# gabrielspmoreira/chameleon_recsys

Hardware: AMD Instinct MI355X
Metric: NAR training sessions/sec (higher is better)
Workload: dtype f32

## Files before the change

### chameleon_recsys_amd/csrc/dm_fused.hip

```cpp
#include "gemm_shared.h"
#include <type_traits>

#define DMF_NT 2
#define DMF_COLS (32 * DMF_NT)
#define DMF_PLANE (DMF_COLS * 128)
#define DMF_HALF (3 * DMF_PLANE)
#define DMF_RED_OFF (2 * DMF_HALF)
#define DMF_RED_BYTES (8 * 4 * DMF_COLS * 4)

static_assert(DMF_NT == 2, "the epilogue packs exactly two tiles' columns per lane");

struct DmfParams {
    const float* dS1; int lds1;
    const __bf16* W; long long w_ps;
    const float* Z2c; const float* pred;
    __bf16* out; long long out_ps;
    const H2Scale* osc;
    const H2Scale* sa; const H2Scale* sw;
    float* dpred; float* b2part;
    int C, BT, NC, PW;
    int out_blocked;
};

__device__ __forceinline__ void dmf_dma_one(unsigned lds, unsigned voff, const u32x4& r) {
    unsigned keep;
    asm volatile(
        "s_nop 4\n\t"
        "s_mov_b32 %0, m0\n\t"
        "s_mov_b32 m0, %1\n\ts_nop 0\n\tbuffer_load_dwordx4 %2, %3, 0 offen lds\n\t"
        "s_mov_b32 m0, %0"
        : "=&s"(keep) : "s"(lds), "v"(voff), "s"(r) : "memory");
}

template <int MODE>
__global__ __launch_bounds__(512) void k_dm_mulpred_fused(DmfParams p) {
    constexpr bool H2 = MODE == 1 || MODE == 3, B16 = MODE == 2, F16P = MODE == 3;
    constexpr int NPL = B16 ? 1 : (F16P ? 2 : 3);
    extern __shared__ __attribute__((aligned(1024))) unsigned char dmf_smem[];
    const int lane = threadIdx.x & 63, wave = __builtin_amdgcn_readfirstlane(threadIdx.x >> 6);
    const int l31 = lane & 31, hh = lane >> 5;
    const int NC = p.NC, C = p.C;
    const int pos0 = blockIdx.x * p.PW;
    const int npos = min(p.PW, p.BT - pos0);
    const int rows_valid = npos * NC;
    const size_t row0 = (size_t)pos0 * NC;
    const int wr0 = 32 * wave;

    bf16x8 AH[8], AM[(B16 || F16P) ? 1 : 8], AL[B16 ? 1 : 8];
    float ginv_a = 1.f, ginv_w = 1.f;
    if constexpr (B16) {
        const __bf16* a16 = reinterpret_cast<const __bf16*>(p.dS1);
        const __amdgpu_buffer_rsrc_t aw = __builtin_amdgcn_make_buffer_rsrc(const_cast<__bf16*>(a16 + row0 * (size_t)p.lds1), 0,
                                                                            (unsigned)((size_t)rows_valid * p.lds1 * 2), 0x00020000);
        const unsigned ao = ((unsigned)(wr0 + l31) * (unsigned)p.lds1 + 8u * hh) * 2u;
#pragma unroll
        for (int s = 0; s < 8; ++s) AH[s] = __builtin_bit_cast(bf16x8, __builtin_amdgcn_raw_buffer_load_b128(aw, ao + 32u * s, 0, 0));
    } else {
        const __amdgpu_buffer_rsrc_t aw = __builtin_amdgcn_make_buffer_rsrc(const_cast<float*>(p.dS1 + row0 * (size_t)p.lds1), 0,
                                                                            (unsigned)((size_t)rows_valid * p.lds1 * 4), 0x00020000);
        const unsigned ao = ((unsigned)(wr0 + l31) * (unsigned)p.lds1 + 8u * hh) * 4u;
        u32x4 x[16];
#pragma unroll
        for (int s = 0; s < 8; ++s) {
            x[2 * s] = __builtin_amdgcn_raw_buffer_load_b128(aw, ao + 64u * s, 0, 0);
            x[2 * s + 1] = __builtin_amdgcn_raw_buffer_load_b128(aw, ao + 64u * s + 16u, 0, 0);
        }
#pragma unroll
        for (int s = 0; s < 8; ++s) {
            const float v[8] = {__uint_as_float(x[2 * s].x), __uint_as_float(x[2 * s].y), __uint_as_float(x[2 * s].z), __uint_as_float(x[2 * s].w),
                                __uint_as_float(x[2 * s + 1].x), __uint_as_float(x[2 * s + 1].y), __uint_as_float(x[2 * s + 1].z),
                                __uint_as_float(x[2 * s + 1].w)};
            if constexpr (F16P) {
                const float sa = p.sa->scale;
#pragma unroll
                for (int e = 0; e < 8; ++e) {
                    _Float16 a, c;
                    split2h(v[e] * sa, a, c);
                    AH[s][e] = __builtin_bit_cast(__bf16, a); AL[s][e] = __builtin_bit_cast(__bf16, c);
                }
            } else {
#pragma unroll
                for (int e = 0; e < 8; ++e) { __bf16 a, b, c; split3(v[e], a, b, c); AH[s][e] = a; AM[s][e] = b; AL[s][e] = c; }
            }
        }
    }
    const __amdgpu_buffer_rsrc_t zw = B16 ?
        __builtin_amdgcn_make_buffer_rsrc(const_cast<__bf16*>(reinterpret_cast<const __bf16*>(p.Z2c) + row0 * (size_t)C), 0,
                                          (unsigned)((size_t)rows_valid * C * 2), 0x00020000) :
        __builtin_amdgcn_make_buffer_rsrc(const_cast<float*>(p.Z2c + row0 * (size_t)C), 0, (unsigned)((size_t)rows_valid * C * 4), 0x00020000);
    __amdgpu_buffer_rsrc_t ow[3];
#pragma unroll
    for (int q = 0; q < 3; ++q)
        ow[q] = __builtin_amdgcn_make_buffer_rsrc(p.out + ((H2 && q == 2) || B16 ? 0 : q) * p.out_ps + row0 * (size_t)C, 0, (unsigned)((size_t)rows_valid * C * 2), 0x00020000);
    const bool oblk = H2 && p.out_blocked != 0;
    const unsigned rin = (unsigned)(row0 & 255), tile_bytes = ((unsigned)C >> 5) * (unsigned)(H2B_BLOCK * 2);
    if (oblk) {
#pragma unroll
        for (int q = 0; q < 2; ++q)
            ow[q] = __builtin_amdgcn_make_buffer_rsrc(p.out + q * p.out_ps + (row0 >> 8) * (size_t)((unsigned)C >> 5) * H2B_BLOCK, 0, 2u * tile_bytes, 0x00020000);
    }
    float osc = 1.f;
    if constexpr (H2) osc = p.osc->scale;
    if constexpr (F16P) { ginv_a = p.sa->inv; ginv_w = p.sw->inv; }

    typedef __attribute__((address_space(3))) unsigned char lds_u8;
    const unsigned lds_base = (unsigned)(unsigned long long)(lds_u8*)dmf_smem;
    u32x4 rw[3];
#pragma unroll
    for (int q = 0; q < 3; ++q) {
        const unsigned long long a = (unsigned long long)(p.W + q * p.w_ps);
        rw[q].x = (unsigned)a; rw[q].y = (unsigned)(a >> 32) & 0xFFFFu; rw[q].z = (unsigned)((size_t)C * 128 * 2); rw[q].w = 0x00020000u;
    }
    unsigned voff;
    {
        const int slot = 8 * wave + (lane >> 3);
        const int piece = (lane & 7) ^ ((slot >> 1) & 7);
        const int col = DMF_NT * (slot & 31) + (slot >> 5);
        voff = (unsigned)(col * 128 + piece * 8) * 2u;
    }
    auto dma_half = [&](int h) {
        const unsigned base = lds_base + (unsigned)(h & 1) * DMF_HALF + (unsigned)wave * 1024u;
        const unsigned add = (unsigned)(((h >> 1) * DMF_COLS) * 128 + (h & 1) * 64) * 2u;
#pragma unroll
        for (int q = 0; q < NPL; ++q) dmf_dma_one(base + (unsigned)q * DMF_PLANE, voff + add, rw[q]);
    };
    unsigned fo[4];
#pragma unroll
    for (int t = 0; t < 4; ++t) fo[t] = (unsigned)(l31 * 128 + (((2 * t + hh) ^ ((l31 >> 1) & 7)) * 16));

    const int pa = wr0 / NC;
    const int bnd = (pa + 1) * NC - wr0;
    const int ntiles = C / DMF_COLS, nhalf = 2 * ntiles;

    dma_half(0);
    dma_half(1);
    floatx16 acc[DMF_NT];
#pragma unroll
    for (int j = 0; j < DMF_NT; ++j)
#pragma unroll
        for (int e = 0; e < 16; ++e) acc[j][e] = 0.f;
    if constexpr (B16) asm volatile("s_waitcnt vmcnt(1)" ::: "memory");
    else if constexpr (F16P) asm volatile("s_waitcnt vmcnt(2)" ::: "memory");
    else asm volatile("s_waitcnt vmcnt(3)" ::: "memory");
    __builtin_amdgcn_fence(__ATOMIC_RELEASE, "workgroup", "local");
    __builtin_amdgcn_s_barrier();
    __builtin_amdgcn_fence(__ATOMIC_ACQUIRE, "workgroup", "local");

    auto mfma_half = [&](auto PARC) {
        constexpr int PAR = decltype(PARC)::value, s0 = PAR * 4;
        const unsigned char* S = dmf_smem + PAR * DMF_HALF;
        __builtin_amdgcn_sched_barrier(0);
#pragma unroll
        for (int t = 0; t < 4; ++t) {
            bf16x8 bh[DMF_NT], bm[DMF_NT], bl[DMF_NT];
#pragma unroll
            for (int j = 0; j < DMF_NT; ++j) {
                bh[j] = *reinterpret_cast<const bf16x8*>(S + fo[t] + j * 4096);
                if constexpr (F16P) {
                    bl[j] = *reinterpret_cast<const bf16x8*>(S + DMF_PLANE + fo[t] + j * 4096);
                } else if constexpr (!B16) {
                    bm[j] = *reinterpret_cast<const bf16x8*>(S + DMF_PLANE + fo[t] + j * 4096);
                    bl[j] = *reinterpret_cast<const bf16x8*>(S + 2 * DMF_PLANE + fo[t] + j * 4096);
                }
            }
            if constexpr (F16P) {
                typedef _Float16 dmf_half8 __attribute__((ext_vector_type(8)));
#pragma unroll
                for (int j = 0; j < DMF_NT; ++j)
                    acc[j] = __builtin_amdgcn_mfma_f32_32x32x16_f16(__builtin_bit_cast(dmf_half8, AL[s0 + t]), __builtin_bit_cast(dmf_half8, bh[j]), acc[j], 0, 0, 0);
#pragma unroll
                for (int j = 0; j < DMF_NT; ++j)
                    acc[j] = __builtin_amdgcn_mfma_f32_32x32x16_f16(__builtin_bit_cast(dmf_half8, AH[s0 + t]), __builtin_bit_cast(dmf_half8, bl[j]), acc[j], 0, 0, 0);
#pragma unroll
                for (int j = 0; j < DMF_NT; ++j)
                    acc[j] = __builtin_amdgcn_mfma_f32_32x32x16_f16(__builtin_bit_cast(dmf_half8, AH[s0 + t]), __builtin_bit_cast(dmf_half8, bh[j]), acc[j], 0, 0, 0);
            } else if constexpr (B16) {
#pragma unroll
                for (int j = 0; j < DMF_NT; ++j) acc[j] = __builtin_amdgcn_mfma_f32_32x32x16_bf16(AH[s0 + t], bh[j], acc[j], 0, 0, 0);
            } else {
#pragma unroll
                for (int j = 0; j < DMF_NT; ++j) acc[j] = __builtin_amdgcn_mfma_f32_32x32x16_bf16(AL[s0 + t], bh[j], acc[j], 0, 0, 0);
#pragma unroll
                for (int j = 0; j < DMF_NT; ++j) acc[j] = __builtin_amdgcn_mfma_f32_32x32x16_bf16(AH[s0 + t], bl[j], acc[j], 0, 0, 0);
#pragma unroll
                for (int j = 0; j < DMF_NT; ++j) acc[j] = __builtin_amdgcn_mfma_f32_32x32x16_bf16(AM[s0 + t], bm[j], acc[j], 0, 0, 0);
#pragma unroll
                for (int j = 0; j < DMF_NT; ++j) acc[j] = __builtin_amdgcn_mfma_f32_32x32x16_bf16(AM[s0 + t], bh[j], acc[j], 0, 0, 0);
#pragma unroll
                for (int j = 0; j < DMF_NT; ++j) acc[j] = __builtin_amdgcn_mfma_f32_32x32x16_bf16(AH[s0 + t], bm[j], acc[j], 0, 0, 0);
#pragma unroll
                for (int j = 0; j < DMF_NT; ++j) acc[j] = __builtin_amdgcn_mfma_f32_32x32x16_bf16(AH[s0 + t], bh[j], acc[j], 0, 0, 0);
            }
        }
    };
    for (int h = 0; h < nhalf; ++h) {
        if (h & 1) mfma_half(std::integral_constant<int, 1>{});
        else mfma_half(std::integral_constant<int, 0>{});
        __builtin_amdgcn_sched_barrier(0);
        asm volatile("s_waitcnt vmcnt(0)" ::: "memory");
        if (h & 1) {
            const int col = (h >> 1) * DMF_COLS + DMF_NT * l31;
            float2 pra = make_float2(0.f, 0.f), prb = pra;
            if (pa < npos) pra = *reinterpret_cast<const float2*>(p.pred + (size_t)(pos0 + pa) * C + col);
            if (pa + 1 < npos) prb = *reinterpret_cast<const float2*>(p.pred + (size_t)(pos0 + pa + 1) * C + col);
            float2 sa = make_float2(0.f, 0.f), sb = sa, ca = sa, cb = sa;
            typedef unsigned int u32x2_t __attribute__((ext_vector_type(2)));
            u32x2_t zz[16];
#pragma unroll
            for (int e = 0; e < 16; ++e) {
                const unsigned r = (unsigned)(wr0 + (e & 3) + 8 * (e >> 2) + 4 * hh);
                if constexpr (B16) {
                    const unsigned u = __builtin_amdgcn_raw_buffer_load_b32(zw, (r * (unsigned)C + (unsigned)col) * 2u, 0, 0);
                    zz[e].x = u << 16; zz[e].y = u & 0xFFFF0000u;
                } else {
                    zz[e] = __builtin_amdgcn_raw_buffer_load_b64(zw, (r * (unsigned)C + (unsigned)col) * 4u, 0, 0);
                }
            }
#pragma unroll
            for (int e = 0; e < 16; ++e) {
                const int rr = (e & 3) + 8 * (e >> 2) + 4 * hh;
                const unsigned r = (unsigned)(wr0 + rr);
                const float2 z = make_float2(__uint_as_float(zz[e].x), __uint_as_float(zz[e].y));
                const bool second = rr >= bnd;
                const float2 pr = second ? prb : pra;
                float2 g = make_float2(acc[0][e], acc[1][e]);
                if constexpr (F16P) { g.x = (g.x * ginv_a) * ginv_w; g.y = (g.y * ginv_a) * ginv_w; }
                if constexpr (B16) { g.x = (float)(__bf16)g.x; g.y = (float)(__bf16)g.y; }
                float2 o;
                o.x = g.x * pr.x * (1.f - z.x * z.x); o.y = g.y * pr.y * (1.f - z.y * z.y);
                if constexpr (B16) {
                    typedef __bf16 bf16x2_t __attribute__((ext_vector_type(2)));
                    bf16x2_t ph; ph[0] = (__bf16)o.x; ph[1] = (__bf16)o.y;
                    __builtin_amdgcn_raw_buffer_store_b32(__builtin_bit_cast(unsigned, ph), ow[0], (r * (unsigned)C + (unsigned)col) * 2u, 0, 0);
                    o.x = (float)ph[0]; o.y = (float)ph[1];
                } else if constexpr (H2) {
                    _Float16 h0, l0, h1, l1;
                    split2h(o.x * osc, h0, l0); split2h(o.y * osc, h1, l1);
                    const unsigned ph = (unsigned)h2_keep_sign(h0, o.x) | ((unsigned)h2_keep_sign(h1, o.y) << 16);
                    const unsigned pl = (unsigned)__builtin_bit_cast(unsigned short, l0) | ((unsigned)__builtin_bit_cast(unsigned short, l1) << 16);
                    unsigned oo = (r * (unsigned)C + (unsigned)col) * 2u;
                    if (oblk) {
                        const unsigned lr = rin + r;
                        oo = (int)r < rows_valid ? (lr >> 8) * tile_bytes + ((unsigned)col >> 5) * (unsigned)(H2B_BLOCK * 2) + (lr & 255u) * 64u + ((unsigned)col & 31u) * 2u
                                                 : 0x80000000u;
                    }
                    __builtin_amdgcn_raw_buffer_store_b32(ph, ow[0], oo, 0, 0);
                    __builtin_amdgcn_raw_buffer_store_b32(pl, ow[1], oo, 0, 0);
                } else {
                    typedef __bf16 bf16x2_t __attribute__((ext_vector_type(2)));
                    bf16x2_t ph, pm, pl;
                    __bf16 a, b, c;
                    split3(o.x, a, b, c); ph[0] = a; pm[0] = b; pl[0] = c;
                    split3(o.y, a, b, c); ph[1] = a; pm[1] = b; pl[1] = c;
                    const unsigned oo = (r * (unsigned)C + (unsigned)col) * 2u;
                    __builtin_amdgcn_raw_buffer_store_b32(__builtin_bit_cast(unsigned, ph), ow[0], oo, 0, 0);
                    __builtin_amdgcn_raw_buffer_store_b32(__builtin_bit_cast(unsigned, pm), ow[1], oo, 0, 0);
                    __builtin_amdgcn_raw_buffer_store_b32(__builtin_bit_cast(unsigned, pl), ow[2], oo, 0, 0);
                }
                const float2 gz = make_float2(g.x * z.x, g.y * z.y);
                sb.x += second ? gz.x : 0.f; sb.y += second ? gz.y : 0.f; cb.x += second ? o.x : 0.f; cb.y += second ? o.y : 0.f;
                sa.x += second ? 0.f : gz.x; sa.y += second ? 0.f : gz.y; ca.x += second ? 0.f : o.x; ca.y += second ? 0.f : o.y;
                acc[0][e] = 0.f; acc[1][e] = 0.f;
            }
            float* red = reinterpret_cast<float*>(dmf_smem + DMF_RED_OFF) + (size_t)wave * (4 * DMF_COLS);
            float2 q[4] = {sa, ca, sb, cb};
#pragma unroll
            for (int i = 0; i < 4; ++i) {
                float2 o;
                o.x = __shfl_xor(q[i].x, 32, 64); o.y = __shfl_xor(q[i].y, 32, 64);
                if (hh == 0) *reinterpret_cast<float2*>(red + i * DMF_COLS + DMF_NT * l31) = make_float2(q[i].x + o.x, q[i].y + o.y);
            }
        }
        __builtin_amdgcn_fence(__ATOMIC_RELEASE, "workgroup", "local");
        __builtin_amdgcn_s_waitcnt(0xc07f);
        __builtin_amdgcn_s_barrier();
        __builtin_amdgcn_fence(__ATOMIC_ACQUIRE, "workgroup", "local");
        if (h & 1) {
            const float* redw = reinterpret_cast<const float*>(dmf_smem + DMF_RED_OFF);
            for (int idx = threadIdx.x; idx < npos * DMF_COLS; idx += 512) {
                const int pl = idx / DMF_COLS, c = idx % DMF_COLS;
                float s = 0.f, cs = 0.f;
                const int w_lo = (pl * NC) >> 5, w_hi = min(7, ((pl + 1) * NC - 1) >> 5);
                for (int w = w_lo; w <= w_hi; ++w) {
                    const int slot = (pl == (32 * w) / NC) ? 0 : 1;
                    s += redw[(size_t)w * (4 * DMF_COLS) + slot * (2 * DMF_COLS) + c];
                    cs += redw[(size_t)w * (4 * DMF_COLS) + slot * (2 * DMF_COLS) + DMF_COLS + c];
                }
                const int colg = (h >> 1) * DMF_COLS + c;
                const float pr = p.pred[(size_t)(pos0 + pl) * C + colg];
                p.dpred[(size_t)(pos0 + pl) * C + colg] = s * (1.f - pr * pr);
                if (p.b2part) p.b2part[(size_t)(pos0 + pl) * C + colg] = cs;
            }
        }
        if (h + 2 < nhalf) dma_half(h + 2);
    }
    asm volatile("s_waitcnt vmcnt(0)" ::: "memory");
}

template <int MODE>
static int dm_mulpred_launch(const float* dS1, int lds1, int K, const void* Wp, long long w_plane_stride, const float* Z2c,
                             const float* pred, int C, int BT, int N, void* dZ2p, long long out_plane_stride, const void* out_scale_rec,
                             float* dpred_pre, float* col_part, void* stream, const void* a_scale_rec = nullptr, const void* w_scale_rec = nullptr,
                             int out_blocked = 0) {
    if (!dS1 || !Wp || !Z2c || !pred || !dZ2p || !dpred_pre || BT < 0 || N < 0 || ((MODE == 1 || MODE == 3) && !out_scale_rec)) return -CHAM_ERR_ARG;
    if (MODE == 3 && (!a_scale_rec || !w_scale_rec || (((uintptr_t)a_scale_rec | (uintptr_t)w_scale_rec) & 3))) return -CHAM_ERR_ARG;
    const int NC = N + 1;
    if (K != 128 || (C % DMF_COLS) || C <= 0 || NC < 32 || NC > 256 || (lds1 & 3) || lds1 < K || (out_plane_stride & 3) || (w_plane_stride & 7))
        return -CHAM_ERR_ARG;
    if (((uintptr_t)dS1 | (uintptr_t)Wp | (uintptr_t)Z2c | (uintptr_t)pred | (uintptr_t)dZ2p) & 15) return -CHAM_ERR_ARG;
    if (out_blocked && ((MODE != 1 && MODE != 3) || (C & 31) || out_plane_stride < (long long)(((size_t)BT * NC + 255) / 256) * (C >> 5) * H2B_BLOCK)) return -CHAM_ERR_ARG;
    if (BT == 0) return CHAM_OK;
    DmfParams p;
    p.out_blocked = out_blocked ? 1 : 0;
    p.dS1 = dS1; p.lds1 = lds1; p.W = reinterpret_cast<const __bf16*>(Wp); p.w_ps = w_plane_stride; p.Z2c = Z2c; p.pred = pred;
    p.out = reinterpret_cast<__bf16*>(dZ2p); p.out_ps = out_plane_stride; p.osc = reinterpret_cast<const H2Scale*>(out_scale_rec);
    p.sa = reinterpret_cast<const H2Scale*>(a_scale_rec); p.sw = reinterpret_cast<const H2Scale*>(w_scale_rec);
    p.dpred = dpred_pre; p.b2part = col_part;
    p.C = C; p.BT = BT; p.NC = NC; p.PW = 256 / NC;
    constexpr int smem = 2 * DMF_HALF + DMF_RED_BYTES;
    auto k = k_dm_mulpred_fused<MODE>;
    CHAM_SET_DYNAMIC_LDS(k, smem);
    hipLaunchKernelGGL(k, dim3((BT + p.PW - 1) / p.PW), dim3(512), smem, (hipStream_t)stream, p);
    CHAM_CHECK_LAUNCH();
    return CHAM_OK;
}

extern "C" int cham_dm_mulpred_p3(const float* dS1, int lds1, int K, const void* Wp, long long w_plane_stride, const float* Z2c,
                                  const float* pred, int C, int BT, int N, void* dZ2p, long long out_plane_stride, float* dpred_pre,
                                  float* col_part, void* stream) {
    return dm_mulpred_launch<0>(dS1, lds1, K, Wp, w_plane_stride, Z2c, pred, C, BT, N, dZ2p, out_plane_stride, nullptr, dpred_pre, col_part, stream);
}

extern "C" int cham_dm_mulpred_h2(const float* dS1, int lds1, int K, const void* Wp, long long w_plane_stride, const float* Z2c,
                                  const float* pred, int C, int BT, int N, void* dZ2p, long long out_plane_stride, const void* out_scale_rec,
                                  float* dpred_pre, float* col_part, void* stream) {
    return dm_mulpred_launch<1>(dS1, lds1, K, Wp, w_plane_stride, Z2c, pred, C, BT, N, dZ2p, out_plane_stride, out_scale_rec, dpred_pre, col_part, stream);
}

extern "C" int cham_dm_mulpred_h2h(const float* dS1, int lds1, int K, const void* Wh, long long w_plane_stride, const void* ds1_scale_rec,
                                   const void* w_scale_rec, const float* Z2c, const float* pred, int C, int BT, int N, void* dZ2p,
                                   long long out_plane_stride, const void* out_scale_rec, float* dpred_pre, float* col_part, void* stream) {
    return dm_mulpred_launch<3>(dS1, lds1, K, Wh, w_plane_stride, Z2c, pred, C, BT, N, dZ2p, out_plane_stride, out_scale_rec, dpred_pre, col_part, stream,
                                ds1_scale_rec, w_scale_rec);
}

extern "C" int cham_dm_mulpred_h2_blk(const float* dS1, int lds1, int K, const void* Wp, long long w_plane_stride, const void* ds1_scale_rec,
                                      const void* w_scale_rec, const float* Z2c, const float* pred, int C, int BT, int N, void* dZ2p,
                                      long long out_plane_stride, const void* out_scale_rec, float* dpred_pre, float* col_part, void* stream) {
    if ((ds1_scale_rec == nullptr) != (w_scale_rec == nullptr)) return -CHAM_ERR_ARG;
    if (ds1_scale_rec)
        return dm_mulpred_launch<3>(dS1, lds1, K, Wp, w_plane_stride, Z2c, pred, C, BT, N, dZ2p, out_plane_stride, out_scale_rec, dpred_pre, col_part, stream,
                                    ds1_scale_rec, w_scale_rec, 1);
    return dm_mulpred_launch<1>(dS1, lds1, K, Wp, w_plane_stride, Z2c, pred, C, BT, N, dZ2p, out_plane_stride, out_scale_rec, dpred_pre, col_part, stream,
                                nullptr, nullptr, 1);
}

extern "C" int cham_dm_mulpred_b16(const void* dS1, int lds1, int K, const void* Ws1b, const void* Z2c, const float* pred, int C, int BT, int N,
                                   void* dZ2c, float* dpred_pre, float* col_part, void* stream) {
    if ((lds1 & 7)) return -CHAM_ERR_ARG;
    return dm_mulpred_launch<2>(reinterpret_cast<const float*>(dS1), lds1, K, Ws1b, 0, reinterpret_cast<const float*>(Z2c), pred, C, BT, N, dZ2c, 0,
                                nullptr, dpred_pre, col_part, stream);
}
```

Baseline: 34460.

## Prefetch Z2/pred tiles during MFMA and defer column sums past next tile

Restructures the fused dZ2 kernel loop per column tile. The Z2c and pred loads are issued before the first MFMA half so their latency overlaps compute instead of stalling after it. The cross-wave column reduction for tile t is deferred to the next iteration's mid-tile barrier, with pred values staged in LDS so the epilogue no longer rereads global memory. It also picks between FMA-contracted and uncontracted forms of the tanh-derivative and split3 residual per element, likely to match the reference rounding. This adds register pressure from holding the prefetched tiles and makes the DMA/barrier ordering more intricate.

```diff
diff --git a/chameleon_recsys_amd/csrc/dm_fused.hip b/chameleon_recsys_amd/csrc/dm_fused.hip
--- a/chameleon_recsys_amd/csrc/dm_fused.hip
+++ b/chameleon_recsys_amd/csrc/dm_fused.hip
@@ -6,7 +6,8 @@
 #define DMF_PLANE (DMF_COLS * 128)
 #define DMF_HALF (3 * DMF_PLANE)
 #define DMF_RED_OFF (2 * DMF_HALF)
-#define DMF_RED_BYTES (8 * 4 * DMF_COLS * 4)
+#define DMF_RED_WAVE (6 * DMF_COLS)
+#define DMF_RED_BYTES (8 * DMF_RED_WAVE * 4)
 
 static_assert(DMF_NT == 2, "the epilogue packs exactly two tiles' columns per lane");
 
@@ -31,6 +32,29 @@
         "s_mov_b32 m0, %0"
         : "=&s"(keep) : "s"(lds), "v"(voff), "s"(r) : "memory");
 }
+
+template <bool FUSED>
+__device__ __forceinline__ float dmf_one_minus_sq(float z) {
+    if constexpr (FUSED) {
+        return __builtin_fmaf(-z, z, 1.f);
+    } else {
+#pragma clang fp contract(off)
+        const float q = z * z;
+        return 1.f - q;
+    }
+}
+__host__ __device__ constexpr bool dmf_tanh_fused(int mode, int e) { return mode == 3 || (mode != 2 && e >= 8); }
+template <bool RESID_FUSED>
+__device__ __forceinline__ void dmf_split3_prod(float x, float t, float& o, __bf16& h, __bf16& m, __bf16& l) {
+#pragma clang fp contract(off)
+    o = x * t;
+    h = (__bf16)o;
+    float r = RESID_FUSED ? __builtin_fmaf(x, t, -(float)h) : o - (float)h;
+    m = (__bf16)r;
+    r -= (float)m;
+    l = (__bf16)r;
+}
+__host__ __device__ constexpr bool dmf_resid_fused(int mode, int e) { return mode == 0 && e < 7; }
 
 template <int MODE>
 __global__ __launch_bounds__(512) void k_dm_mulpred_fused(DmfParams p) {
@@ -193,41 +217,87 @@
             }
         }
     };
-    for (int h = 0; h < nhalf; ++h) {
-        if (h & 1) mfma_half(std::integral_constant<int, 1>{});
-        else mfma_half(std::integral_constant<int, 0>{});
+    const __amdgpu_buffer_rsrc_t pw = __builtin_amdgcn_make_buffer_rsrc(const_cast<float*>(p.pred + (size_t)pos0 * C), 0,
+                                                                        (unsigned)((size_t)npos * C * 4), 0x00020000);
+    typedef unsigned int u32x2_t __attribute__((ext_vector_type(2)));
+    typedef std::conditional_t<B16, unsigned, u32x2_t> dmf_zraw;
+    dmf_zraw zz[16];
+    u32x2_t pz[2];
+    auto load_tile = [&](int t) {
+        const unsigned col = (unsigned)(t * DMF_COLS + DMF_NT * l31);
+#pragma unroll
+        for (int e = 0; e < 16; ++e) {
+            const unsigned r = (unsigned)(wr0 + (e & 3) + 8 * (e >> 2) + 4 * hh);
+            if constexpr (B16) zz[e] = __builtin_amdgcn_raw_buffer_load_b32(zw, (r * (unsigned)C + col) * 2u, 0, 0);
+            else zz[e] = __builtin_amdgcn_raw_buffer_load_b64(zw, (r * (unsigned)C + col) * 4u, 0, 0);
+        }
+#pragma unroll
+        for (int i = 0; i < 2; ++i) pz[i] = __builtin_amdgcn_raw_buffer_load_b64(pw, ((unsigned)(pa + i) * (unsigned)C + col) * 4u, 0, 0);
+    };
+    auto sync_stage = [&]() {
+        __builtin_amdgcn_fence(__ATOMIC_RELEASE, "workgroup", "local");
+        __builtin_amdgcn_s_waitcnt(0xc07f);
+        __builtin_amdgcn_s_barrier();
+        __builtin_amdgcn_fence(__ATOMIC_ACQUIRE, "workgroup", "local");
+    };
+    auto col_sums = [&](int t) {
+        const float* redw = reinterpret_cast<const float*>(dmf_smem + DMF_RED_OFF);
+        for (int idx = threadIdx.x; idx < npos * DMF_COLS; idx += 512) {
+            const int pl = idx / DMF_COLS, c = idx % DMF_COLS;
+            float s = 0.f, cs = 0.f;
+            const int w_lo = (pl * NC) >> 5, w_hi = min(7, ((pl + 1) * NC - 1) >> 5);
+            for (int w = w_lo; w <= w_hi; ++w) {
+                const int slot = (pl == (32 * w) / NC) ? 0 : 1;
+                s += redw[(size_t)w * DMF_RED_WAVE + slot * (2 * DMF_COLS) + c];
+                cs += redw[(size_t)w * DMF_RED_WAVE + slot * (2 * DMF_COLS) + DMF_COLS + c];
+            }
+            const int colg = t * DMF_COLS + c;
+            const float pr = redw[(size_t)w_lo * DMF_RED_WAVE + (4 + ((pl == (32 * w_lo) / NC) ? 0 : 1)) * DMF_COLS + c];
+            p.dpred[(size_t)(pos0 + pl) * C + colg] = s * dmf_one_minus_sq<true>(pr);
+            if (p.b2part) p.b2part[(size_t)(pos0 + pl) * C + colg] = cs;
+        }
+    };
+    for (int t = 0; t < ntiles; ++t) {
+        load_tile(t);
+        mfma_half(std::integral_constant<int, 0>{});
         __builtin_amdgcn_sched_barrier(0);
-        asm volatile("s_waitcnt vmcnt(0)" ::: "memory");
-        if (h & 1) {
-            const int col = (h >> 1) * DMF_COLS + DMF_NT * l31;
-            float2 pra = make_float2(0.f, 0.f), prb = pra;
-            if (pa < npos) pra = *reinterpret_cast<const float2*>(p.pred + (size_t)(pos0 + pa) * C + col);
-            if (pa + 1 < npos) prb = *reinterpret_cast<const float2*>(p.pred + (size_t)(pos0 + pa + 1) * C + col);
+        asm volatile("s_waitcnt vmcnt(18)" ::: "memory");
+        sync_stage();
+        if (t > 0) col_sums(t - 1);
+        if (2 * t + 2 < nhalf) dma_half(2 * t + 2);
+        mfma_half(std::integral_constant<int, 1>{});
+        __builtin_amdgcn_sched_barrier(0);
+        asm volatile("s_waitcnt vmcnt(0)"
+                     : "+v"(zz[0]), "+v"(zz[1]), "+v"(zz[2]), "+v"(zz[3]), "+v"(zz[4]), "+v"(zz[5]), "+v"(zz[6]), "+v"(zz[7]), "+v"(zz[8]), "+v"(zz[9]),
+                       "+v"(zz[10]), "+v"(zz[11]), "+v"(zz[12]), "+v"(zz[13]), "+v"(zz[14]), "+v"(zz[15]), "+v"(pz[0]), "+v"(pz[1])
+                     :: "memory");
+        sync_stage();
+        if (2 * t + 3 < nhalf) dma_half(2 * t + 3);
+        {
+            const int col = t * DMF_COLS + DMF_NT * l31;
+            const float2 pra = make_float2(__uint_as_float(pz[0].x), __uint_as_float(pz[0].y));
+            const float2 prb = make_float2(__uint_as_float(pz[1].x), __uint_as_float(pz[1].y));
             float2 sa = make_float2(0.f, 0.f), sb = sa, ca = sa, cb = sa;
-            typedef unsigned int u32x2_t __attribute__((ext_vector_type(2)));
-            u32x2_t zz[16];
-#pragma unroll
-            for (int e = 0; e < 16; ++e) {
-                const unsigned r = (unsigned)(wr0 + (e & 3) + 8 * (e >> 2) + 4 * hh);
-                if constexpr (B16) {
-                    const unsigned u = __builtin_amdgcn_raw_buffer_load_b32(zw, (r * (unsigned)C + (unsigned)col) * 2u, 0, 0);
-                    zz[e].x = u << 16; zz[e].y = u & 0xFFFF0000u;
-                } else {
-                    zz[e] = __builtin_amdgcn_raw_buffer_load_b64(zw, (r * (unsigned)C + (unsigned)col) * 4u, 0, 0);
-                }
-            }
+            unsigned rin_t = rin;
+            if constexpr (MODE == 1) asm volatile("" : "+s"(rin_t));
 #pragma unroll
             for (int e = 0; e < 16; ++e) {
                 const int rr = (e & 3) + 8 * (e >> 2) + 4 * hh;
                 const unsigned r = (unsigned)(wr0 + rr);
-                const float2 z = make_float2(__uint_as_float(zz[e].x), __uint_as_float(zz[e].y));
+                float2 z;
+                if constexpr (B16) z = make_float2(__uint_as_float(zz[e] << 16), __uint_as_float(zz[e] & 0xFFFF0000u));
+                else z = make_float2(__uint_as_float(zz[e].x), __uint_as_float(zz[e].y));
                 const bool second = rr >= bnd;
                 const float2 pr = second ? prb : pra;
                 float2 g = make_float2(acc[0][e], acc[1][e]);
                 if constexpr (F16P) { g.x = (g.x * ginv_a) * ginv_w; g.y = (g.y * ginv_a) * ginv_w; }
                 if constexpr (B16) { g.x = (float)(__bf16)g.x; g.y = (float)(__bf16)g.y; }
                 float2 o;
-                o.x = g.x * pr.x * (1.f - z.x * z.x); o.y = g.y * pr.y * (1.f - z.y * z.y);
+                const bool fz = dmf_tanh_fused(MODE, e);
+                const float2 tz = fz ? make_float2(dmf_one_minus_sq<true>(z.x), dmf_one_minus_sq<true>(z.y))
+                                     : make_float2(dmf_one_minus_sq<false>(z.x), dmf_one_minus_sq<false>(z.y));
+                const float2 gp = make_float2(g.x * pr.x, g.y * pr.y);
+                o.x = gp.x * tz.x; o.y = gp.y * tz.y;
                 if constexpr (B16) {
                     typedef __bf16 bf16x2_t __attribute__((ext_vector_type(2)));
                     bf16x2_t ph; ph[0] = (__bf16)o.x; ph[1] = (__bf16)o.y;
@@ -240,7 +310,7 @@
                     const unsigned pl = (unsigned)__builtin_bit_cast(unsigned short, l0) | ((unsigned)__builtin_bit_cast(unsigned short, l1) << 16);
                     unsigned oo = (r * (unsigned)C + (unsigned)col) * 2u;
                     if (oblk) {
-                        const unsigned lr = rin + r;
+                        const unsigned lr = rin_t + r;
                         oo = (int)r < rows_valid ? (lr >> 8) * tile_bytes + ((unsigned)col >> 5) * (unsigned)(H2B_BLOCK * 2) + (lr & 255u) * 64u + ((unsigned)col & 31u) * 2u
                                                  : 0x80000000u;
                     }
@@ -250,8 +320,11 @@
                     typedef __bf16 bf16x2_t __attribute__((ext_vector_type(2)));
                     bf16x2_t ph, pm, pl;
                     __bf16 a, b, c;
-                    split3(o.x, a, b, c); ph[0] = a; pm[0] = b; pl[0] = c;
-                    split3(o.y, a, b, c); ph[1] = a; pm[1] = b; pl[1] = c;
+                    const bool fr = dmf_resid_fused(MODE, e);
+                    if (fr) dmf_split3_prod<true>(gp.x, tz.x, o.x, a, b, c); else dmf_split3_prod<false>(gp.x, tz.x, o.x, a, b, c);
+                    ph[0] = a; pm[0] = b; pl[0] = c;
+                    if (fr) dmf_split3_prod<true>(gp.y, tz.y, o.y, a, b, c); else dmf_split3_prod<false>(gp.y, tz.y, o.y, a, b, c);
+                    ph[1] = a; pm[1] = b; pl[1] = c;
                     const unsigned oo = (r * (unsigned)C + (unsigned)col) * 2u;
                     __builtin_amdgcn_raw_buffer_store_b32(__builtin_bit_cast(unsigned, ph), ow[0], oo, 0, 0);
                     __builtin_amdgcn_raw_buffer_store_b32(__builtin_bit_cast(unsigned, pm), ow[1], oo, 0, 0);
@@ -262,7 +335,7 @@
                 sa.x += second ? 0.f : gz.x; sa.y += second ? 0.f : gz.y; ca.x += second ? 0.f : o.x; ca.y += second ? 0.f : o.y;
                 acc[0][e] = 0.f; acc[1][e] = 0.f;
             }
-            float* red = reinterpret_cast<float*>(dmf_smem + DMF_RED_OFF) + (size_t)wave * (4 * DMF_COLS);
+            float* red = reinterpret_cast<float*>(dmf_smem + DMF_RED_OFF) + (size_t)wave * DMF_RED_WAVE;
             float2 q[4] = {sa, ca, sb, cb};
 #pragma unroll
             for (int i = 0; i < 4; ++i) {
@@ -270,30 +343,14 @@
                 o.x = __shfl_xor(q[i].x, 32, 64); o.y = __shfl_xor(q[i].y, 32, 64);
                 if (hh == 0) *reinterpret_cast<float2*>(red + i * DMF_COLS + DMF_NT * l31) = make_float2(q[i].x + o.x, q[i].y + o.y);
             }
-        }
-        __builtin_amdgcn_fence(__ATOMIC_RELEASE, "workgroup", "local");
-        __builtin_amdgcn_s_waitcnt(0xc07f);
-        __builtin_amdgcn_s_barrier();
-        __builtin_amdgcn_fence(__ATOMIC_ACQUIRE, "workgroup", "local");
-        if (h & 1) {
-            const float* redw = reinterpret_cast<const float*>(dmf_smem + DMF_RED_OFF);
-            for (int idx = threadIdx.x; idx < npos * DMF_COLS; idx += 512) {
-                const int pl = idx / DMF_COLS, c = idx % DMF_COLS;
-                float s = 0.f, cs = 0.f;
-                const int w_lo = (pl * NC) >> 5, w_hi = min(7, ((pl + 1) * NC - 1) >> 5);
-                for (int w = w_lo; w <= w_hi; ++w) {
-                    const int slot = (pl == (32 * w) / NC) ? 0 : 1;
-                    s += redw[(size_t)w * (4 * DMF_COLS) + slot * (2 * DMF_COLS) + c];
-                    cs += redw[(size_t)w * (4 * DMF_COLS) + slot * (2 * DMF_COLS) + DMF_COLS + c];
-                }
-                const int colg = (h >> 1) * DMF_COLS + c;
-                const float pr = p.pred[(size_t)(pos0 + pl) * C + colg];
-                p.dpred[(size_t)(pos0 + pl) * C + colg] = s * (1.f - pr * pr);
-                if (p.b2part) p.b2part[(size_t)(pos0 + pl) * C + colg] = cs;
-            }
-        }
-        if (h + 2 < nhalf) dma_half(h + 2);
-    }
+            if (hh == 0) {
+                *reinterpret_cast<float2*>(red + 4 * DMF_COLS + DMF_NT * l31) = pra;
+                *reinterpret_cast<float2*>(red + 5 * DMF_COLS + DMF_NT * l31) = prb;
+            }
+        }
+    }
+    sync_stage();
+    col_sums(ntiles - 1);
     asm volatile("s_waitcnt vmcnt(0)" ::: "memory");
 }
 
```

New measurement: 34970 (median of 6 runs). +1.5%, better.
